# DRCL-USC/Hector_Simulation

Hardware: AMD Instinct MI355X
Metric: MPC QP solves/sec (horizon=10, 2 contacts) (higher is better)
Workload: dtype f32 assembly / f64 solve; 1 GPU; 2-contact standing randomized MPC ticks, horizon 10, reduced QP up to 120x160; records and forces device-resident in/out; two batches of the same instances one 5 ms tick apart, solved alternately; batch_per_gpu=8192, global_batch=8192, horizon=10, contacts=2, launch_streams=2, world=1, launcher=python (single process), devices_visible=1, parallelism=single GPU

## Files before the change

### hector_simulation_amd/csrc/hmpc_kernel.h

```cpp
#pragma once
#include <stddef.h>
#include <stdint.h>

#include <type_traits>
#include <utility>

#ifndef HMPC_REFINE
#define HMPC_REFINE 1
#endif

#include "hmpc_math.h"

#include "hmpc_kernel_args.h"
#include "hmpc_record.h"
#include "hmpc_front.h"
#include "hmpc_schur_tiles.h"
#include "hmpc_matvec_index.h"

namespace hmpc {
#ifdef HMPC_PROFILE
struct Prof {
  long long pt, pt0, acc[NPROF];
  __device__ __forceinline__ Prof() : pt(clock64()), pt0(pt) {
    for (int i = 0; i < NPROF; ++i) acc[i] = 0;
  }
  __device__ __forceinline__ void mark(int ph) {
    const long long n = clock64();
    acc[ph] += n - pt;
    pt = n;
  }
  __device__ __forceinline__ void flush(const KernelArgs &args, int inst) {
    if (threadIdx.x == 0 && args.prof) {
      acc[P_TOTAL] = clock64() - pt0;
      for (int i = 0; i < NPROF; ++i) args.prof[(size_t)inst * NPROF + i] = acc[i];
    }
  }
};
#define PROF_MARK(ph) prof.mark(ph)
#define PROF_FLUSH() prof.flush(args, inst)
#else
struct Prof {};
#define PROF_MARK(ph)
#define PROF_FLUSH()
#endif
#define PROF_DECL Prof prof
}

namespace hmpc {

constexpr int GS = 6;


template <int NMAX, int HMAX, int NT, int QCAP, int NC = 2, int BPT = 1>
struct Smem {
  static constexpr int U = 6 * NC;
  static constexpr int PS = 13 * U;
  static constexpr int NG = NMAX / GS;
  static constexpr int MMAX = NG * 8;
  static constexpr int NW = NT / 64;
  static constexpr bool EGLOBAL = (QCAP == 0);
  static constexpr int QMAX = EGLOBAL ? NMAX : QCAP;
  static constexpr int EP_LDS = EGLOBAL ? 1 : QMAX * (QMAX + 1) / 2;
  static constexpr int RECW = rec_stride(NC, HMAX) / 4;
  static constexpr bool FULLBLK = (HMAX <= 10 && NMAX >= 120);
  static constexpr int HSP = (NC == 3 && BPT == 2) ? 2 : 1;
  static constexpr int HS_D0 = 3;
  static constexpr int hs_dlo(int p) { return p <= 0 ? 0 : (p >= HSP ? HMAX : HS_D0); }
  static constexpr int hs_off(int d, int h) { return d * h - d * (d - 1) / 2; }
  static constexpr int HS_BLOCKS = (HSP == 1) ? HMAX * (HMAX + 1) / 2
                                              : (hs_off(HS_D0, HMAX) > HMAX * (HMAX + 1) / 2 - hs_off(HS_D0, HMAX)
                                                     ? hs_off(HS_D0, HMAX) : HMAX * (HMAX + 1) / 2 - hs_off(HS_D0, HMAX));
  static constexpr int STH = (BPT == 2) ? 2 : 1;
  static constexpr int STR = NG / STH;
  static_assert(NG % 2 == 0 && (STH == 1 || STH == 2), "the staged mat-vec sums two groups of NG/2 source leg-steps");

  double g[NMAX];
  double Cn[NC][8][6];
  double ub7[NG];
  double relax;
  double sc7[NG];
  unsigned char vstep[NMAX], vcomp[NMAX];
  unsigned char o2s[NMAX], s2o[NMAX];
  unsigned short sinfo[NMAX];
  static constexpr bool MFS2 = (NMAX == 120 && NT == 256 && BPT == 1 && NC == 2);
  static constexpr bool MFS3 = (NMAX == 180 && NT == 256 && BPT == 2 && NC == 3) ||
                               (NMAX == 240 && NT == 512 && BPT == 2 && NC == 2 && QCAP != 0);
  signed char kexp[(MFS2 || MFS3) ? 16 * ((NMAX + 15) / 16) : 1];
  unsigned char rmap[U * HMAX];
  unsigned char ls_leg[NG], ls_step[NG];
  int n, m, nls, pad0;

  struct Asm {
    uint32_t rec[RECW];
    float sc[10][2];
    float sc234[2][2];
    float rpy[3];
    float ypsc[4];
    float Acd[169], Bcd[PS], x0[13], W[13], Fc[8 * NC * U];
    float Apow[2 * 169];
    float Phi[HMAX * PS];
    float e[13 * HMAX];
    unsigned char pre_nl[HMAX], pre_nv[HMAX], pre_st[HMAX];
    float Hs[FULLBLK ? HS_BLOCKS * U * U + 64 : (NMAX / 2) * (NMAX + 1)];
  };
  struct Rec {
    double val, raw, cn[6];
    int idx, side, pad1, pad2;
  };
  struct Sol {
    alignas(16) double x[NMAX], xu[NMAX], z[NMAX], w[NMAX];
    alignas(16) double ST[STR][NMAX + 2];
    alignas(16) double piv[2][NMAX];
    double pd[2];
    double u[NMAX], d[NMAX], r[NMAX], col[NMAX];
    double redv[NW], redw[NW];
    double gamma;
    int redi[NW];
    int wcount[NW];
    Rec rec[NW];
    alignas(8) signed char act[MMAX];
    alignas(8) unsigned char slot[MMAX];
    unsigned char flpc[MMAX];
    typedef typename std::conditional<(MMAX > 256), unsigned short, unsigned char>::type row_t;
    row_t Wrow[NMAX];
    double Ep[EP_LDS];
  };
  union {
    Asm a;
    Sol s;
  } u;
  int2 hadr[MFS2 ? NMAX : 1];
};

template <class SM, int NT, int BPT>
struct SpillLayout {
  typedef typename SM::Sol SolT;
  static constexpr size_t A_BYTES = offsetof(SolT, ST);
  static constexpr size_t B_OFF = offsetof(SolT, piv), B_BYTES = offsetof(SolT, Ep) - offsetof(SolT, piv);
  static constexpr size_t E_OFF = A_BYTES + B_BYTES;
  static constexpr size_t M_BYTES = (size_t)BPT * GS * GS * NT * sizeof(double);
  static constexpr size_t stride_for(int rows) { return (E_OFF + (size_t)rows * (rows + 1) / 2 * sizeof(double) + M_BYTES + 255) / 256 * 256; }
  static_assert(A_BYTES % 8 == 0 && B_OFF % 8 == 0 && B_BYTES % 8 == 0, "copied as 8-byte words");
};

template <int NMAX>
__device__ __forceinline__ int hs_index(int i, int j) {
  const bool first = 2 * i < NMAX;
  return (first ? i : NMAX - 1 - i) * (NMAX + 1) + (first ? j - i : j + 1);
}
__device__ __forceinline__ int uni(int v) { return __builtin_amdgcn_readfirstlane(v); }
__device__ __forceinline__ double uni_d(double v) {
  const int lo = __builtin_amdgcn_readfirstlane(__double2loint(v)), hi = __builtin_amdgcn_readfirstlane(__double2hiint(v));
  return __hiloint2double(hi, lo);
}
__device__ __forceinline__ bool ub(bool c) { return __builtin_amdgcn_readfirstlane((int)c) != 0; }

template <int CTRL>
__device__ __forceinline__ double dpp_move(double v) {
  int lo = __double2loint(v), hi = __double2hiint(v);
  lo = __builtin_amdgcn_update_dpp(lo, lo, CTRL, 0xF, 0xF, false);
  hi = __builtin_amdgcn_update_dpp(hi, hi, CTRL, 0xF, 0xF, false);
  return __hiloint2double(hi, lo);
}
__device__ __forceinline__ double dpp_xor1(double v) { return dpp_move<0xB1>(v); }
__device__ __forceinline__ double dpp_xor2(double v) { return dpp_move<0x4E>(v); }
__device__ __forceinline__ double dmin(double a, double b) { return b < a ? b : a; }
__device__ __forceinline__ double readlane_d(double v, int lane) {
  int lo = __builtin_amdgcn_readlane(__double2loint(v), lane), hi = __builtin_amdgcn_readlane(__double2hiint(v), lane);
  return __hiloint2double(hi, lo);
}
__device__ __forceinline__ double wave_min(double v) {
  v = dmin(v, dpp_move<0xB1>(v));
  v = dmin(v, dpp_move<0x4E>(v));
  v = dmin(v, dpp_move<0x141>(v));
  v = dmin(v, dpp_move<0x140>(v));
  const double r0 = readlane_d(v, 0), r1 = readlane_d(v, 16), r2 = readlane_d(v, 32), r3 = readlane_d(v, 48);
  return dmin(dmin(r0, r1), dmin(r2, r3));
}

}
#ifndef HMPC_EARLY_HANDOVER_MARGIN
#define HMPC_EARLY_HANDOVER_MARGIN 8
#endif
#ifndef HMPC_READD_LIMIT
#define HMPC_READD_LIMIT 6
#endif
#ifndef HMPC_CONT_ITER_BUDGET
#define HMPC_CONT_ITER_BUDGET 128
#endif
#ifndef HMPC_CONT_ROUNDS
#define HMPC_CONT_ROUNDS 4
#endif
namespace hmpc {
constexpr int MFS_GT = 4;
constexpr int MFS_PST_PAD = 18;

template <int NMAX, int HMAX, int NT, int QCAP, int NC, int BPT, Role ROLE, bool ASM_ONLY = false>
struct VariantTraits {
  using SM = Smem<NMAX, HMAX, NT, QCAP, NC, BPT>;
  static constexpr bool WALK_SHAPE = NT == 128;
  static constexpr bool HANDOVER_SHAPE = SM::MFS2;
  static constexpr bool THREE_CONTACT = NC == 3;
  static constexpr bool WIDE_SHAPE = NMAX == 240;
  static constexpr bool EIGHT_WAVES = NT >= 512;
  static constexpr bool EGLOBAL = SM::EGLOBAL;
  static constexpr bool NO_OVERFLOW = EGLOBAL || QCAP >= NMAX;
  static constexpr bool THREE_WAVES = BPT == 1 && !EIGHT_WAVES && sizeof(SM) * (size_t)(3 * 256 / NT) <= (size_t)160 * 1024;
  static constexpr int WAVES_PER_EU = THREE_WAVES ? 3 : 2;
  static constexpr bool LAZY = BPT == 2, LAZY_IDX = LAZY || (HANDOVER_SHAPE && ROLE != Role::SAFE);
  static constexpr bool GATHER_ONCE = !(WIDE_SHAPE && ROLE == Role::SAFE);

  static constexpr bool SWEEP = ROLE == Role::SWEEP;
  static constexpr bool SAVES = !ASM_ONLY && HANDOVER_SHAPE && (ROLE == Role::FAST || SWEEP);
  static constexpr size_t SPILL_STRIDE = (SAVES && ROLE == Role::FAST) ? SpillLayout<SM, NT, BPT>::stride_for(QCAP) : 0;
  static constexpr bool RESUMES = ROLE == Role::CONT;
  static constexpr bool LISTED = ROLE == Role::SAFE || RESUMES;
  static constexpr bool LONGRUN = ROLE == Role::SAFE && NO_OVERFLOW, REGULARISES = LONGRUN, REFRESHES = LONGRUN;
  static constexpr bool ANTICYCLE = (LONGRUN || RESUMES) && HMPC_READD_LIMIT > 0;
  static constexpr bool ITER_LONG = ROLE == Role::SAFE || NO_OVERFLOW || WIDE_SHAPE;
  static constexpr bool READS_FRONT = !ASM_ONLY && ROLE == Role::FAST && NC == 2 && BPT == 1;

  static constexpr bool MFMA_SWEEP = !ASM_ONLY && HANDOVER_SHAPE && ROLE != Role::SAFE;
  static constexpr bool MFMA_SWEEP3 = !ASM_ONLY && SM::MFS3 && ROLE == Role::FAST;
  static constexpr int MFS3_NTG = (NMAX + 15) / 16;
  static constexpr bool MFS3_ROW_PASSES = false;
  static constexpr bool SCHUR_ROW_PASSES = !WIDE_SHAPE;

  static constexpr int BLOCK_ROUNDS = WALK_SHAPE ? 1 : THREE_CONTACT ? 3 : 2;
  static constexpr int CONT_ROUNDS = HMPC_CONT_ROUNDS;
  static constexpr bool BLOCK_FRICTION = !WALK_SHAPE;
  static constexpr int BLOCK_MIN_NEW = THREE_CONTACT ? 2 : 3;
  static constexpr int NTGS = RESUMES ? 6 : EIGHT_WAVES ? 5 : THREE_CONTACT ? 4 : 3;
  static constexpr bool SCHUR_MFMA = !LONGRUN && !WALK_SHAPE && SM::QMAX >= 16 * NTGS;
  static constexpr int EPT = 5;
  static constexpr int KBMAX = SCHUR_MFMA ? 16 * NTGS : EIGHT_WAVES ? 71 : WALK_SHAPE ? 34 : 45;

  static_assert(sizeof(SM) <= 160 * 1024, "LDS budget of a gfx950 CU");
  static_assert(BPT == 1 || EIGHT_WAVES || sizeof(SM) <= 80 * 1024, "two workgroups per CU");
  static_assert(SM::NG * (SM::NG + 1) / 2 <= BPT * NT && SM::MMAX <= NT && NMAX <= NT, "threads per block / constraint row / variable");
  static_assert((SCHUR_MFMA || KBMAX * (KBMAX + 1) / 2 <= EPT * NT) && KBMAX <= SM::QMAX, "block start capacity");
  static_assert(!ASM_ONLY || ROLE == Role::FAST, "assembly-only debug kernels belong to the FAST rows");
  static_assert(!SWEEP || (!ASM_ONLY && BPT == 1 && NC == 2 && !EGLOBAL), "command sweeps: the fast two-contact shapes");
  static_assert(!(HANDOVER_SHAPE && (ROLE == Role::FAST || SWEEP)) || QCAP < HMPC_QCAP_CONT, "a FAST / SWEEP variant on the hand-over shape saves a full working set for the CONT variant to resume: its capacity (HMPC_QCAP_FAST) must be below HMPC_QCAP_CONT");
  static_assert(!RESUMES || (HANDOVER_SHAPE && QCAP >= HMPC_QCAP_CONT && QCAP < NMAX), "a CONT variant exists only on the hand-over shape, with at least HMPC_QCAP_CONT rows and fewer than variables");
  static_assert(!(HANDOVER_SHAPE && ROLE == Role::SAFE) || NO_OVERFLOW, "the SAFE variant of the hand-over shape ends the chain: its working set cannot overflow");
};

template <bool LAZY, class F>
struct LazyInt {
  int v;
  F f;
  __device__ __forceinline__ operator int() const {
// ... 663 lines not shown
  constexpr int NG = SM::NG, U = SM::U, PS = SM::PS, C8 = 8 * NC;
  auto &A = S.u.a;
  const int tid = threadIdx.x;
  (void)prof;
  const float *rf = reinterpret_cast<const float *>(A.rec);
  const unsigned char *gait = reinterpret_cast<const unsigned char *>(A.rec + RL::NF + 12 * h);
  const float *in_p = rf + RL::P, *in_v = rf + RL::V, *in_q = rf + RL::Q, *in_w = rf + RL::W, *in_r = rf + RL::R,
              *in_ja = rf + RL::JA, *in_wt = rf + RL::WT;
  auto fz_cap = [&](int c) __attribute__((always_inline)) -> float { return (NC == 3 && c == 2) ? rf[RL::FMH] : args.f_max; };
  bool from_front = false;
  if constexpr (FRONT) from_front = args.front != nullptr;
  if (from_front) {
    if constexpr (FRONT) front_scatter<NMAX, HMAX, NT, QCAP, NC, BPT>(S, args, inst, h);
    __syncthreads();
    PROF_MARK(P_A1);
  } else {
  {
    constexpr int L_ROLL = (NT >= 256) ? 65 : 65, L_PITCH = (NT >= 256) ? 128 : 66, L_YAW = (NT >= 256) ? 192 : 12;
    if (tid < 12) {
      const float ang = front_trig_angle(in_ja, tid);
      double s, c;
      det_sincos((double)ang, s, c);
      float *dst = (tid < 10) ? A.sc[tid] : A.sc234[tid - 10];
      dst[0] = (float)s;
      dst[1] = (float)c;
    } else if (tid == L_ROLL || tid == L_PITCH || tid == L_YAW) {
      if (tid == L_ROLL) {
        A.rpy[0] = front_euler_angle<0>(in_q);
      } else if (tid == L_PITCH) {
        const float pitch = front_euler_angle<1>(in_q);
        A.rpy[1] = pitch;
        double s, c;
        det_sincos((double)pitch, s, c);
        A.ypsc[2] = (float)c;
        A.ypsc[3] = (float)s;
      } else {
        const float yaw = front_euler_angle<2>(in_q);
        A.rpy[2] = yaw;
        double s, c;
        det_sincos((double)yaw, s, c);
        A.ypsc[0] = (float)c;
        A.ypsc[1] = (float)s;
      }
    } else if (tid == 64) {
      int nv, nl;
      front_prefix<NC>(gait, h, fz_cap, A.pre_nl, A.pre_nv, A.pre_st, nv, nl);
      S.n = nv;
      S.nls = nl;
      S.m = 8 * nl;
    }
    for (int t = tid; t < 169; t += NT) A.Acd[t] = (t % 14 == 0) ? 1.0f : 0.0f;
    for (int t = tid; t < PS; t += NT) A.Bcd[t] = 0.0f;
    for (int t = tid; t < C8 * U; t += NT) A.Fc[t] = 0.0f;
    for (int t = tid; t < U * h; t += NT) S.rmap[t] = 255;
    if (tid == 0) S.relax = args.relax, S.pad0 = 0;
  }
  __syncthreads();
  PROF_MARK(P_A1);

  if (tid == 0) {
    float Rbi_dt[9], Iinv_dt[9], blk_dt[NC][9];
    front_body<NC>(in_q, A.ypsc, in_r, args.Ib, args.dt, Rbi_dt, Iinv_dt, blk_dt);
    for (int i = 0; i < 3; ++i) {
      A.x0[i] = A.rpy[i];
      A.x0[3 + i] = in_p[i];
      A.x0[6 + i] = in_w[i];
      A.x0[9 + i] = in_v[i];
    }
    A.x0[12] = args.gravity;
    const float dt = args.dt;
    for (int i = 0; i < 3; ++i)
      for (int j = 0; j < 3; ++j) A.Acd[i * 13 + 6 + j] = Rbi_dt[i * 3 + j];
    for (int i = 0; i < 3; ++i) A.Acd[(3 + i) * 13 + 9 + i] = 0.0f + dt * 1.0f;
    A.Acd[11 * 13 + 12] = 0.0f + dt * -1.0f;
    const float inv_m = args.inv_mass;
    for (int leg = 0; leg < NC; ++leg) {
      for (int i = 0; i < 3; ++i)
        for (int j = 0; j < 3; ++j) {
          A.Bcd[(6 + i) * U + 3 * leg + j] = blk_dt[leg][i * 3 + j];
          A.Bcd[(6 + i) * U + 3 * NC + 3 * leg + j] = Iinv_dt[i * 3 + j];
        }
      for (int i = 0; i < 3; ++i) A.Bcd[(9 + i) * U + 3 * leg + i] = dt * inv_m;
    }
    for (int s = 0; s < 12; ++s) A.W[s] = in_wt[s];
    A.W[12] = 0.0f;
  }
  {
    const int leg_lane0 = (NT >= 256) ? 128 : 64, leg_lane1 = (NT >= 256) ? 192 : 65, leg_lane2 = (NC == 3) ? (NT >= 512 ? 256 : 96) : -1;
    if (tid == leg_lane0 || tid == leg_lane1 || tid == leg_lane2) {
      const int leg = (tid == leg_lane0) ? 0 : (tid == leg_lane1 ? 1 : 2);
      const float mu = args.mu_inst ? args.mu_inst[inst] : args.mu;
      float t0[3], t1[3], flt[3], flh[3];
      front_foot<NC>(in_q, A.sc, A.sc234, leg, args.lt, args.lh , rf + RL::RH, t0, t1, flt, flh);
      float *row = A.Fc + (8 * leg) * U;
      const int cf = 3 * leg, cmo = 3 * NC + 3 * leg;
      row[0 * U + cf + 0] = -mu, row[0 * U + cf + 2] = 1.0f;
      row[1 * U + cf + 0] = mu, row[1 * U + cf + 2] = 1.0f;
      row[2 * U + cf + 1] = -mu, row[2 * U + cf + 2] = 1.0f;
      row[3 * U + cf + 1] = mu, row[3 * U + cf + 2] = 1.0f;
      for (int j = 0; j < 3; ++j) {
        row[4 * U + cmo + j] = t0[j];
        row[5 * U + cf + j] = flt[j];
        row[5 * U + cmo + j] = t1[j];
        row[6 * U + cf + j] = flh[j];
        row[6 * U + cmo + j] = (leg != 1) ? -t1[j] : t1[j];
      }
      row[7 * U + cf + 2] = 2.0f;
      for (int rr = 0; rr < 8; ++rr)
        for (int k = 0; k < 3; ++k) {
          S.Cn[leg][rr][k] = (double)row[rr * U + cf + k];
          S.Cn[leg][rr][3 + k] = (double)row[rr * U + cmo + k];
        }
    }
  }
  }
  if (args.ext_Fc) {
    __syncthreads();
    const float *xf = args.ext_Fc + (size_t)inst * C8 * U;
    for (int t = tid; t < C8 * U; t += NT) A.Fc[t] = xf[t];
    for (int t = tid; t < NC * 8 * 6; t += NT) {
      const int leg = t / 48, rr = (t / 6) % 8, k = t % 6;
      S.Cn[leg][rr][k] = (double)xf[(8 * leg + rr) * U + ((k < 3) ? 3 * leg + k : 3 * NC + 3 * leg + k - 3)];
    }
  }
  {
    const int nl_tot = S.nls;
    if (tid >= 64 && tid < 128 && nl_tot <= NG) {
      for (int it = tid - 64; it < 3 * NC * h; it += 64) {
        const int i = it / (3 * NC), leg = (it / 3) % NC, k = it % 3;
        const int st = A.pre_st[i];
        if (st & (1 << leg)) {
          const int nst = __popc(st), rank = __popc(st & ((1 << leg) - 1));
          const int e = A.pre_nl[i] + rank, nv = A.pre_nv[i];
          const int oF = nv + 3 * rank + k, oM = nv + 3 * nst + 3 * rank + k;
          S.vstep[oF] = (unsigned char)i, S.vcomp[oF] = (unsigned char)(3 * leg + k);
          S.vstep[oM] = (unsigned char)i, S.vcomp[oM] = (unsigned char)(3 * NC + 3 * leg + k);
          S.o2s[oF] = (unsigned char)(GS * e + k), S.s2o[GS * e + k] = (unsigned char)oF;
          S.o2s[oM] = (unsigned char)(GS * e + 3 + k), S.s2o[GS * e + 3 + k] = (unsigned char)oM;
          S.sinfo[GS * e + k] = (unsigned short)(i | ((3 * leg + k) << 8));
          S.sinfo[GS * e + 3 + k] = (unsigned short)(i | ((3 * NC + 3 * leg + k) << 8));
          S.rmap[U * i + 3 * leg + k] = (unsigned char)(GS * e + k);
          S.rmap[U * i + 3 * NC + 3 * leg + k] = (unsigned char)(GS * e + 3 + k);
          if (k == 0) {
            S.ls_leg[e] = (unsigned char)leg;
            S.ls_step[e] = (unsigned char)i;
            const double u7 = (double)(fz_cap(leg) * (float)gait[NC * i + leg]);
            S.ub7[e] = u7;
            S.sc7[e] = (u7 > 1.0) ? 1.0 / u7 : 1.0;
          }
        }
      }
    }
  }
  for (int t = tid; t < 169; t += NT) A.Apow[t] = (t % 14 == 0) ? 1.0f : 0.0f;
  __syncthreads();
}

template <int NMAX, int HMAX, int NT, int QCAP, int NC, int BPT>
__device__ __forceinline__ void stage_a_chains(Smem<NMAX, HMAX, NT, QCAP, NC, BPT> &S, const KernelArgs &args, const int inst, const int h, const int n, Prof &prof) {
  using SM = Smem<NMAX, HMAX, NT, QCAP, NC, BPT>;
  using RL = RecLayout<NC>;
  constexpr int U = SM::U, PS = SM::PS;
  auto &A = S.u.a;
  const int tid = threadIdx.x;
  (void)prof;
  const float *in_traj = reinterpret_cast<const float *>(A.rec) + RL::NF;
  constexpr int NITEM = 169 + PS + 13, NTRIP = (NITEM + NT - 1) / NT;
  int it_p[NTRIP][4];
  const float *it_c[NTRIP][4];
  int it_kind[NTRIP], it_out[NTRIP];
#pragma unroll
  for (int u = 0; u < NTRIP; ++u) {
    const int t = tid + u * NT;
    int row, cs, m0, m1, m2, m3, kind, out;
    const float *cf;
    if (t < 169) {
      const int i = t / 13, j = t % 13, pad = (j == 12) ? 0 : 12;
      const bool w3 = j >= 6 && j < 9;
      row = i, cf = A.Acd + j, cs = 13, kind = 0, out = t;
      m0 = w3 ? 0 : ((j >= 9 && j < 12) ? j - 6 : (j == 12 ? 11 : pad));
      m1 = w3 ? 1 : pad, m2 = w3 ? 2 : pad, m3 = j;
    } else if (t < 169 + PS) {
      const int rem = t - 169, i = rem / U, j = rem % U;
      row = i, cf = A.Bcd + j, cs = U, kind = 1, out = rem;
      m0 = 6, m1 = 7, m2 = 8, m3 = (j < 3 * NC) ? 9 + j % 3 : 0;
    } else {
      const int s = (t < NITEM) ? t - (169 + PS) : 0;
      row = s, cf = A.x0, cs = 1, kind = (t < NITEM) ? 2 : 3, out = s;
      m0 = s;
      m1 = (s < 3) ? 6 : ((s < 5) ? s + 6 : ((s == 5) ? 11 : ((s == 11) ? 12 : 0)));
      m2 = (s < 3) ? 7 : ((s == 5) ? 12 : 0);
      m3 = (s < 3) ? 8 : 0;
    }
    it_p[u][0] = row * 13 + m0, it_p[u][1] = row * 13 + m1, it_p[u][2] = row * 13 + m2, it_p[u][3] = row * 13 + m3;
    it_c[u][0] = cf + m0 * cs, it_c[u][1] = cf + m1 * cs, it_c[u][2] = cf + m2 * cs, it_c[u][3] = cf + m3 * cs;
    it_kind[u] = kind, it_out[u] = out;
  }
  for (int k = 0; k <= h; ++k) {
    const float *Pk = A.Apow + (k & 1) * 169;
    float *Pn = A.Apow + ((k + 1) & 1) * 169;
#pragma unroll
    for (int u = 0; u < NTRIP; ++u) {
      float acc = ffma(Pk[it_p[u][0]], *it_c[u][0], 0.0f);
      acc = ffma(Pk[it_p[u][1]], *it_c[u][1], acc);
      acc = ffma(Pk[it_p[u][2]], *it_c[u][2], acc);
      acc = ffma(Pk[it_p[u][3]], *it_c[u][3], acc);
      const int kind = it_kind[u], out = it_out[u];
      if (kind == 0) {
        if (k < h) Pn[out] = acc;
      } else if (kind == 1) {
        if (k < h) {
          A.Phi[k * PS + out] = acc;
        }
      } else if (kind == 2 && k >= 1) {
        const float xd = (out < 12) ? in_traj[12 * (k - 1) + out] : 0.0f;
        A.e[13 * (k - 1) + out] = acc - xd;
      }
    }
    __syncthreads();
  }

  PROF_MARK(P_ASM);
  if (tid < n) {
    const int a = S.vstep[tid], c = S.vcomp[tid];
    float acc = 0.0f;
    for (int i = a; i < h; ++i) {
      const float *sp = A.Phi + (i - a) * PS + c;
      const float *ep = A.e + 13 * i;
#pragma unroll
      for (int s = 0; s < 13; ++s) acc = ffma(A.W[s] * sp[s * U], ep[s], acc);
    }
    S.g[S.o2s[tid]] = args.ext_g ? (double)args.ext_g[(size_t)inst * args.ext_ld + tid] : (double)(2.0f * acc);
  }
  PROF_MARK(P_G);
}

template <int NMAX, int HMAX, int NT, int QCAP, int NC, int BPT>
__device__ __forceinline__ void stage_output(Smem<NMAX, HMAX, NT, QCAP, NC, BPT> &S, const KernelArgs &args, const int inst, const int h, const int n,
                                             const int q, const int iters, const int code, const bool capped, const bool slot_consumed) {
  using SM = Smem<NMAX, HMAX, NT, QCAP, NC, BPT>;
  constexpr int U = SM::U, C8 = 8 * NC;
  auto &Q = S.u.s;
  const int tid = threadIdx.x;
  int t_out = tid;
  if constexpr (BPT == 2) asm volatile("" : "+v"(t_out));
  for (int t = t_out; t < U * h; t += NT) {
    const int rmp = S.rmap[t];
    const double xv = (rmp == 255) ? 0.0 : Q.x[rmp];
    args.forces[(size_t)inst * U * h + t] = (float)xv;
    if (args.x64) args.x64[(size_t)inst * U * h + t] = xv;
  }
  if (args.wset) {
    for (int t = tid; t < C8 * h; t += NT) {
      const int st = t / C8, cc = (t % C8) >> 3, rr = t & 7;
      const int rmp = S.rmap[U * st + 3 * cc];
      signed char av = 0;
      if (rmp != 255 && code == S_OK) av = Q.act[8 * (rmp / GS) + rr];
      args.wset[(size_t)inst * C8 * h + t] = av;
    }
  }
  if (tid == 0) {
    if (slot_consumed) args.spill_slot[inst] = -1;
    args.status[inst] = (uint32_t)code | ((uint32_t)(iters & 0xfff) << 8) | ((uint32_t)(q & 0xfff) << 20);
    if ((code == S_WORKSET || code == S_MAXITER || code == S_INFEASIBLE || code == S_KKT) && !capped) {
      if (args.flagged) atomicAdd(args.flagged, 1u);
      if (args.flag_count) {
        const unsigned int k = atomicAdd(args.flag_count, 1u);
        if ((int)k < args.flag_cap) args.flag_list[k] = inst;
      }
    }
    if (args.obj64) {
      double o = 0.0;
      for (int i = 0; i < n; ++i) o = dfma(0.5 * S.g[i], Q.x[i], o);
      for (int j = 0; j < q; ++j) {
        const int c = Q.Wrow[j], rr = c & 7;
        const double sj = (double)Q.act[c];
        double bnd = (sj > 0) ? 0.0 : ((rr == 4) ? (double)0.01f : (rr == 7 ? S.ub7[c >> 3] : 0.0));
        const double rl = S.relax;
        if (rl != 0.0) {
          const double fr = 0.6180339887498949 * (double)(c + 1);
          const double dl = rl * (1.0 + (fr - __builtin_floor(fr)));
          bnd = (sj > 0) ? -dl : bnd + dl * ((rr == 7 && bnd > 1.0) ? bnd : 1.0);
        }
        o = dfma(0.5 * Q.u[j], sj * bnd, o);
      }
      args.obj64[inst] = o;
    }
  }
}

template <int NMAX, int HMAX, int NT, int QCAP, bool ASM_ONLY, int NC, int BPT, bool TILES_FROM_STAGING>
__device__ __forceinline__ void stage_h(Smem<NMAX, HMAX, NT, QCAP, NC, BPT> &S, const KernelArgs &args, const int inst, const int h, const int n, const int ng,
                                        BlockOwner<Smem<NMAX, HMAX, NT, QCAP, NC, BPT>::NG, NT, BPT> &bo, double (&a)[BPT][GS][GS]) {
  using SM = Smem<NMAX, HMAX, NT, QCAP, NC, BPT>;
  using RL = RecLayout<NC>;
  constexpr int NW = SM::NW, U = SM::U, PS = SM::PS;
  constexpr bool MFMA_SWEEP = TILES_FROM_STAGING;
  auto &A = S.u.a;
  const int tid = threadIdx.x, wv = uni(tid >> 6);
  const auto ln = lazy_int<(BPT == 2)>([](int t) { return t & 63; });
  const float *in_al = reinterpret_cast<const float *>(A.rec) + RL::AL;
  auto E0 = [&](const int s) __attribute__((always_inline)) -> int { return bo.E0(s); };
  auto E1 = [&](const int s) __attribute__((always_inline)) -> int { return bo.E1(s); };
  auto I0 = [&](const int s) __attribute__((always_inline)) -> int { return bo.I0(s); };
  auto J0 = [&](const int s) __attribute__((always_inline)) -> int { return bo.J0(s); };
  auto OWN = [&](const int s) __attribute__((always_inline)) -> bool { return bo.OWN(s); };
  auto DIAG = [&](const int s) __attribute__((always_inline)) -> bool { return bo.DIAG(s); };
  auto own_blocks = [&]() __attribute__((always_inline)) { bo.assign(); };
  if constexpr (SM::FULLBLK) {
    typedef float f4 __attribute__((ext_vector_type(4)));
    const int l15 = ln & 15, kq = ln >> 4;
    const float wq0 = A.W[kq], wq1 = A.W[kq + 4], wq2 = A.W[kq + 8];
    constexpr int TB = (U + 15) / 16, UU = U * U;
    constexpr int HB_SPARE = SM::HS_BLOCKS * UU;
    static_assert(HB_SPARE + 64 <= (int)(sizeof(A.Hs) / sizeof(float)), "spare words of the padding lanes lie inside Hs");
    const int nchain = h * TB * TB;
    struct Chain {
      bool live, av, bv;
      int d, len, ra, cb;
      int off[4], vm[4];
      float al[4];
    };
    constexpr bool CHAIN_BALANCE = TB == 1 && SM::HSP == 1 && NW == 4 && HMAX <= 10;
    int chain_lim = nchain, chain_dlo = 0;
    auto setup = [&](int idx, Chain &C) __attribute__((always_inline)) {
      int cidx = idx;
      bool alive = idx < chain_lim;
      if constexpr (CHAIN_BALANCE) {
        const int dd = (idx < 4) ? idx : ((idx < 8) ? 11 - idx : ((idx < 10) ? 99 : idx - 2));
        alive = dd < h;
        cidx = dd;
      }
      C.live = alive;
      const int ci = C.live ? cidx : 0;
      C.d = ci / (TB * TB);
      const int ti = (ci / TB) % TB, tj = ci % TB;
      C.len = C.live ? h - C.d : 0;
      C.ra = 16 * ti + l15, C.cb = 16 * tj + l15;
      C.av = C.live && C.ra < U, C.bv = C.live && C.cb < U;
#pragma unroll
      for (int rg = 0; rg < 4; ++rg) {
        const int r = 16 * ti + 4 * kq + rg;
        const bool ok = C.bv && r < U;
        C.vm[rg] = ok ? 1 : 0;
        C.off[rg] = ok ? r * U + C.cb : HB_SPARE + ln;
        C.al[rg] = (ok && C.d == 0 && r == C.cb) ? in_al[r] : 0.0f;
      }
    };
    auto fetch = [&](const Chain &C, int j, float (&o)[6]) __attribute__((always_inline)) {
      const bool la = C.av && j < C.len, lb = C.bv && j < C.len;
      const float *pa = A.Phi + (la ? (j + C.d) * PS + C.ra : 0) + kq * U;
      const float *pb = A.Phi + (lb ? j * PS + C.cb : 0) + kq * U;
      const float a0 = wq0 * pa[0], a1 = wq1 * pa[4 * U], a2 = wq2 * pa[8 * U];
      const float b0 = pb[0], b1 = pb[4 * U], b2 = pb[8 * U];
      o[0] = la ? a0 : 0.0f, o[1] = la ? a1 : 0.0f, o[2] = la ? a2 : 0.0f;
      o[3] = lb ? b0 : 0.0f, o[4] = lb ? b1 : 0.0f, o[5] = lb ? b2 : 0.0f;
    };
    auto store = [&](const Chain &C, int m, const f4 &acc) __attribute__((always_inline)) {
      if (!(C.live && m < C.len)) return;
      const int sb = h - 1 - m, sa = sb - C.d;
      const int base = (SM::hs_off(C.d, h) - SM::hs_off(chain_dlo, h) + sa) * UU;
#pragma unroll
      for (int rg = 0; rg < 4; ++rg) A.Hs[base * C.vm[rg] + C.off[rg]] = 2.0f * (acc[rg] + C.al[rg]);
    };
    auto run_chains = [&](const int idx_lo, const int idx_hi_in) __attribute__((always_inline)) {
    const int idx_hi = CHAIN_BALANCE ? 12 : idx_hi_in;
    for (int idx = idx_lo + wv; idx < idx_hi; idx += 2 * NW) {
      Chain C0, C1;
      setup(idx, C0);
      setup(idx + NW, C1);
      const int steps = C0.len;
      f4 acc0 = {0.0f, 0.0f, 0.0f, 0.0f}, acc1 = {0.0f, 0.0f, 0.0f, 0.0f};
      float c0[6], c1[6], n0[6] = {0.f, 0.f, 0.f, 0.f, 0.f, 0.f}, n1[6] = {0.f, 0.f, 0.f, 0.f, 0.f, 0.f};
// ... 1698 lines not shown
```

Before: 8.113 million QP solves/s.

## Compute sparse A powers in registers once, then build Phi and e in parallel

Replaces the per-step loop that advanced the full 13x13 A-power matrix in shared memory, with a block-wide sync per horizon step, by a compact scheme. Sixteen lanes propagate only the 14 structurally nonzero entries of the power matrix in registers and write each power to a small table. After one sync, all threads compute Phi and the state-error chains for every step from that table, batching KB steps of loads. This removes h-1 barriers and redundant work, at the cost of a serial chain on a few lanes and more complex index encoding.

```diff
diff --git a/hector_simulation_amd/csrc/hmpc_chains.h b/hector_simulation_amd/csrc/hmpc_chains.h
--- /dev/null
+++ b/hector_simulation_amd/csrc/hmpc_chains.h
@@ -0,0 +1,151 @@
+#pragma once
+#include "hmpc_math.h"
+
+namespace hmpc {
+
+constexpr int CH_LIVE = 14, CH_ONE = 14, CH_ZERO = 15, CH_SLOTS = 16;
+
+constexpr int chains_live_row(const int L) { return L < 9 ? L / 3 : (L == 9 ? 3 : (L == 10 ? 4 : (L < 13 ? 5 : 11))); }
+constexpr int chains_live_col(const int L) { return L < 9 ? 6 + L % 3 : (L < 12 ? L : 12); }
+constexpr int chains_slot(const int r, const int m) {
+  return (r < 3 && m >= 6 && m < 9) ? 3 * r + m - 6
+         : ((r == 3 || r == 4) && m == r + 6) ? r + 6
+         : (r == 5 && (m == 11 || m == 12)) ? m
+         : (r == 11 && m == 12) ? 13
+         : (r == m ? CH_ONE : CH_ZERO);
+}
+constexpr int chains_partner(const int L) { return L == 11 ? 12 : (L == 12 ? 11 : L); }
+constexpr float chains_identity_slot(const int t) { return t == CH_ONE ? 1.0f : 0.0f; }
+
+constexpr int chains_power_term(const int j, const int t) {
+  const int pad = (j == 12) ? 0 : 12;
+  const bool w3 = j >= 6 && j < 9;
+  return t == 3 ? j : (w3 ? t : (t == 0 ? ((j >= 9 && j < 12) ? j - 6 : (j == 12 ? 11 : pad)) : pad));
+}
+constexpr int chains_phi_term(const int c, const int t) { return t < 3 ? 6 + t : (c < 3 ? 9 + c : 0); }
+constexpr int chains_e_term(const int s, const int t) {
+  return t == 0 ? s
+         : t == 1 ? ((s < 3) ? 6 : ((s < 5) ? s + 6 : ((s == 5) ? 11 : ((s == 11) ? 12 : 0))))
+         : t == 2 ? ((s < 3) ? 7 : ((s == 5) ? 12 : 0))
+                  : ((s < 3) ? 8 : 0);
+}
+
+typedef unsigned long long chains_word;
+constexpr chains_word chains_pack(int (*f)(int)) {
+  chains_word w = 0;
+  for (int i = 0; i < 16; ++i) w |= (chains_word)(f(i) & 15) << (4 * i);
+  return w;
+}
+__device__ __forceinline__ int chains_entry(const chains_word w, const int i) { return (int)(w >> (4 * i)) & 15; }
+template <int T> constexpr int chains_lane_term(const int L) { return chains_power_term(chains_live_col(L), T); }
+template <int T> constexpr int chains_lane_slot(const int L) { return chains_slot(chains_live_row(L), chains_lane_term<T>(L)); }
+template <int T> constexpr int chains_e_term_of(const int s) { return chains_e_term(s, T); }
+template <int T> constexpr int chains_e_slot_of(const int s) { return chains_slot(s, chains_e_term(s, T)); }
+template <int T, int C> constexpr int chains_phi_slot_of(const int i) { return chains_slot(i, chains_phi_term(C, T)); }
+
+__device__ __forceinline__ unsigned chains_bits(const float x) { return __builtin_bit_cast(unsigned, x); }
+__device__ __forceinline__ float chains_float(const unsigned b) { return __builtin_bit_cast(float, b); }
+
+__device__ __forceinline__ float chains_chain4(const float (&p)[4], const float (&c)[4]) {
+  float acc = ffma(p[0], c[0], 0.0f);
+  acc = ffma(p[1], c[1], acc);
+  acc = ffma(p[2], c[2], acc);
+  return ffma(p[3], c[3], acc);
+}
+
+constexpr bool chains_power_shape_ok() {
+  for (int L = 0; L < CH_LIVE; ++L) {
+    const int i = chains_live_row(L), j = chains_live_col(L);
+    if (chains_slot(i, chains_power_term(j, 3)) != L) return false;
+    for (int t = 0; t < 3; ++t) {
+      const int s = chains_slot(i, chains_power_term(j, t));
+      if (s < CH_LIVE && (s == L || s != chains_partner(L))) return false;
+    }
+  }
+  return true;
+}
+static_assert(chains_power_shape_ok(), "a power lane carries its own entry and its partner's, nothing else");
+struct ChainsPowerLane {
+  float f[2][4];
+  unsigned other[2][3];
+  unsigned one[2][3];
+  float v[2];
+};
+template <int T>
+__device__ __forceinline__ void chains_power_setup_term(ChainsPowerLane &P, const int w, const int Lw, const int Lo, const float *Acd) {
+  constexpr chains_word TERM = chains_pack(&chains_lane_term<T>), SLOT = chains_pack(&chains_lane_slot<T>), COL = chains_pack(&chains_live_col);
+  P.f[w][T] = Acd[chains_entry(TERM, Lw) * 13 + chains_entry(COL, Lw)];
+  if constexpr (T < 3) {
+    const int s = chains_entry(SLOT, Lw);
+    P.other[w][T] = (s == Lo) ? ~0u : 0u;
+    P.one[w][T] = (s == CH_ONE) ? chains_bits(1.0f) : 0u;
+  }
+}
+__device__ __forceinline__ void chains_power_setup(ChainsPowerLane &P, const int L, const float *Acd) {
+  const int Lp = ((L == 11) | (L == 12)) ? (L ^ 7) : L;
+  static_assert(chains_partner(11) == (11 ^ 7) && chains_partner(12) == (12 ^ 7) && chains_partner(13) == 13 && chains_partner(0) == 0, "");
+#pragma unroll
+  for (int w = 0; w < 2; ++w) {
+    const int Lw = w ? Lp : L, Lo = w ? L : Lp;
+    chains_power_setup_term<0>(P, w, Lw, Lo, Acd);
+    chains_power_setup_term<1>(P, w, Lw, Lo, Acd);
+    chains_power_setup_term<2>(P, w, Lw, Lo, Acd);
+    chains_power_setup_term<3>(P, w, Lw, Lo, Acd);
+    P.v[w] = 0.0f;
+  }
+}
+__device__ __forceinline__ void chains_power_step(ChainsPowerLane &P) {
+  const unsigned vb[2] = {chains_bits(P.v[0]), chains_bits(P.v[1])};
+  float nv[2];
+#pragma unroll
+  for (int w = 0; w < 2; ++w) {
+    float p[4];
+#pragma unroll
+    for (int t = 0; t < 3; ++t) p[t] = chains_float((vb[1 - w] & P.other[w][t]) | P.one[w][t]);
+    p[3] = P.v[w];
+    nv[w] = chains_chain4(p, P.f[w]);
+  }
+  P.v[0] = nv[0], P.v[1] = nv[1];
+}
+
+struct ChainsItem {
+  int s[4];
+  float c[4];
+};
+template <int T>
+__device__ __forceinline__ void chains_phi_item_term(ChainsItem &it, const int i, const int j, const int c, const int U, const float *Bcd) {
+  constexpr chains_word S0 = chains_pack(&chains_phi_slot_of<T, 0>), S1 = chains_pack(&chains_phi_slot_of<T, 1>),
+                        S2 = chains_pack(&chains_phi_slot_of<T, 2>), S3 = chains_pack(&chains_phi_slot_of<T, 3>);
+  const chains_word sw = (T < 3) ? S0 : (c == 0 ? S0 : (c == 1 ? S1 : (c == 2 ? S2 : S3)));
+  const int m = (T < 3) ? 6 + T : (c < 3 ? 9 + c : 0);
+  it.s[T] = chains_entry(sw, i);
+  it.c[T] = Bcd[m * U + j];
+}
+template <int NC>
+__device__ __forceinline__ void chains_phi_item(ChainsItem &it, const int r, const float *Bcd) {
+  constexpr int U = 6 * NC;
+  const int i = r / U, j = r % U, c = (j < 3 * NC) ? j % 3 : 3;
+  static_assert(chains_phi_term(0, 3) == 9 && chains_phi_term(2, 3) == 11 && chains_phi_term(3, 3) == 0 && chains_phi_term(3, 1) == 7, "the m of chains_phi_item_term");
+  chains_phi_item_term<0>(it, i, j, c, U, Bcd);
+  chains_phi_item_term<1>(it, i, j, c, U, Bcd);
+  chains_phi_item_term<2>(it, i, j, c, U, Bcd);
+  chains_phi_item_term<3>(it, i, j, c, U, Bcd);
+}
+template <int T>
+__device__ __forceinline__ void chains_e_item_term(ChainsItem &it, const int s, const float *x0) {
+  constexpr chains_word TERM = chains_pack(&chains_e_term_of<T>), SLOT = chains_pack(&chains_e_slot_of<T>);
+  it.s[T] = chains_entry(SLOT, s);
+  it.c[T] = x0[chains_entry(TERM, s)];
+}
+__device__ __forceinline__ void chains_e_item(ChainsItem &it, const int s, const float *x0) {
+  chains_e_item_term<0>(it, s, x0);
+  chains_e_item_term<1>(it, s, x0);
+  chains_e_item_term<2>(it, s, x0);
+  chains_e_item_term<3>(it, s, x0);
+}
+__device__ __forceinline__ float chains_item_value(const ChainsItem &it, const float *pw) {
+  const float p[4] = {pw[it.s[0]], pw[it.s[1]], pw[it.s[2]], pw[it.s[3]]};
+  return chains_chain4(p, it.c);
+}
+
+}
diff --git a/hector_simulation_amd/csrc/hmpc_kernel.h b/hector_simulation_amd/csrc/hmpc_kernel.h
--- a/hector_simulation_amd/csrc/hmpc_kernel.h
+++ b/hector_simulation_amd/csrc/hmpc_kernel.h
@@ -13,6 +13,7 @@
 
 #include "hmpc_kernel_args.h"
 #include "hmpc_record.h"
+#include "hmpc_chains.h"
 #include "hmpc_front.h"
 #include "hmpc_schur_tiles.h"
 #include "hmpc_matvec_index.h"
@@ -97,7 +98,7 @@
     float rpy[3];
     float ypsc[4];
     float Acd[169], Bcd[PS], x0[13], W[13], Fc[8 * NC * U];
-    float Apow[2 * 169];
+    float Pw[(HMAX + 1) * CH_SLOTS];
     float Phi[HMAX * PS];
     float e[13 * HMAX];
     unsigned char pre_nl[HMAX], pre_nv[HMAX], pre_st[HMAX];
@@ -1067,7 +1068,7 @@
       }
     }
   }
-  for (int t = tid; t < 169; t += NT) A.Apow[t] = (t % 14 == 0) ? 1.0f : 0.0f;
+  if (tid < CH_SLOTS) A.Pw[tid] = chains_identity_slot(tid);
   __syncthreads();
 }
 
@@ -1080,60 +1081,59 @@
   const int tid = threadIdx.x;
   (void)prof;
   const float *in_traj = reinterpret_cast<const float *>(A.rec) + RL::NF;
-  constexpr int NITEM = 169 + PS + 13, NTRIP = (NITEM + NT - 1) / NT;
-  int it_p[NTRIP][4];
-  const float *it_c[NTRIP][4];
-  int it_kind[NTRIP], it_out[NTRIP];
+  constexpr int PSE = (PS + 63) / 64 * 64, NITEM = PSE + 13, NTRIP = (NITEM + NT - 1) / NT, KB = 5;
+  static_assert(HMAX % KB == 0, "phase F reads the powers KB at a time, up to Pw[HMAX]");
+  ChainsItem it[NTRIP];
 #pragma unroll
   for (int u = 0; u < NTRIP; ++u) {
     const int t = tid + u * NT;
-    int row, cs, m0, m1, m2, m3, kind, out;
-    const float *cf;
-    if (t < 169) {
-      const int i = t / 13, j = t % 13, pad = (j == 12) ? 0 : 12;
-      const bool w3 = j >= 6 && j < 9;
-      row = i, cf = A.Acd + j, cs = 13, kind = 0, out = t;
-      m0 = w3 ? 0 : ((j >= 9 && j < 12) ? j - 6 : (j == 12 ? 11 : pad));
-      m1 = w3 ? 1 : pad, m2 = w3 ? 2 : pad, m3 = j;
-    } else if (t < 169 + PS) {
-      const int rem = t - 169, i = rem / U, j = rem % U;
-      row = i, cf = A.Bcd + j, cs = U, kind = 1, out = rem;
-      m0 = 6, m1 = 7, m2 = 8, m3 = (j < 3 * NC) ? 9 + j % 3 : 0;
-    } else {
-      const int s = (t < NITEM) ? t - (169 + PS) : 0;
-      row = s, cf = A.x0, cs = 1, kind = (t < NITEM) ? 2 : 3, out = s;
-      m0 = s;
-      m1 = (s < 3) ? 6 : ((s < 5) ? s + 6 : ((s == 5) ? 11 : ((s == 11) ? 12 : 0)));
-      m2 = (s < 3) ? 7 : ((s == 5) ? 12 : 0);
-      m3 = (s < 3) ? 8 : 0;
-    }
-    it_p[u][0] = row * 13 + m0, it_p[u][1] = row * 13 + m1, it_p[u][2] = row * 13 + m2, it_p[u][3] = row * 13 + m3;
-    it_c[u][0] = cf + m0 * cs, it_c[u][1] = cf + m1 * cs, it_c[u][2] = cf + m2 * cs, it_c[u][3] = cf + m3 * cs;
-    it_kind[u] = kind, it_out[u] = out;
-  }
-  for (int k = 0; k <= h; ++k) {
-    const float *Pk = A.Apow + (k & 1) * 169;
-    float *Pn = A.Apow + ((k + 1) & 1) * 169;
-#pragma unroll
-    for (int u = 0; u < NTRIP; ++u) {
-      float acc = ffma(Pk[it_p[u][0]], *it_c[u][0], 0.0f);
-      acc = ffma(Pk[it_p[u][1]], *it_c[u][1], acc);
-      acc = ffma(Pk[it_p[u][2]], *it_c[u][2], acc);
-      acc = ffma(Pk[it_p[u][3]], *it_c[u][3], acc);
-      const int kind = it_kind[u], out = it_out[u];
-      if (kind == 0) {
-        if (k < h) Pn[out] = acc;
-      } else if (kind == 1) {
-        if (k < h) {
-          A.Phi[k * PS + out] = acc;
-        }
-      } else if (kind == 2 && k >= 1) {
-        const float xd = (out < 12) ? in_traj[12 * (k - 1) + out] : 0.0f;
-        A.e[13 * (k - 1) + out] = acc - xd;
-      }
-    }
-    __syncthreads();
-  }
+    if (t < PS) chains_phi_item<NC>(it[u], t, A.Bcd);
+    else chains_e_item(it[u], (t >= PSE && t < NITEM) ? t - PSE : 0, A.x0);
+  }
+  if (tid < CH_SLOTS) {
+    ChainsPowerLane P;
+    chains_power_setup(P, tid < CH_LIVE ? tid : 0, A.Acd);
+    for (int k = 0; k < h; ++k) {
+      chains_power_step(P);
+      A.Pw[(k + 1) * CH_SLOTS + tid] = (tid < CH_LIVE) ? P.v[0] : chains_identity_slot(tid);
+    }
+  }
+  __syncthreads();
+#pragma unroll
+  for (int u = 0; u < NTRIP; ++u) {
+    const int t = tid + u * NT;
+    if (t < PS) {
+      for (int k0 = 0; k0 < h; k0 += KB) {
+        float p[KB][4];
+#pragma unroll
+        for (int kk = 0; kk < KB; ++kk)
+#pragma unroll
+          for (int tt = 0; tt < 4; ++tt) p[kk][tt] = A.Pw[(k0 + kk) * CH_SLOTS + it[u].s[tt]];
+#pragma unroll
+        for (int kk = 0; kk < KB; ++kk) {
+          const float acc = chains_chain4(p[kk], it[u].c);
+          if (k0 + kk < h) A.Phi[(k0 + kk) * PS + t] = acc;
+        }
+      }
+    } else if (t >= PSE && t < NITEM) {
+      const int s = t - PSE;
+      for (int k0 = 0; k0 < h; k0 += KB) {
+        float p[KB][4], xd[KB];
+#pragma unroll
+        for (int kk = 0; kk < KB; ++kk) {
+#pragma unroll
+          for (int tt = 0; tt < 4; ++tt) p[kk][tt] = A.Pw[(k0 + kk + 1) * CH_SLOTS + it[u].s[tt]];
+          xd[kk] = (s < 12) ? in_traj[12 * (k0 + kk) + s] : 0.0f;
+        }
+#pragma unroll
+        for (int kk = 0; kk < KB; ++kk) {
+          const float acc = chains_chain4(p[kk], it[u].c);
+          if (k0 + kk < h) A.e[13 * (k0 + kk) + s] = acc - xd[kk];
+        }
+      }
+    }
+  }
+  __syncthreads();
 
   PROF_MARK(P_ASM);
   if (tid < n) {
```

Result: faster. 8.407 million QP solves/s (median of 6 runs) (+3.6%).
